# rdevooght/sequence-based-recommendations

Hardware: AMD Instinct MI355X
Metric: user-sequences/sec training (ML-1M shape, seq200 b256) at 1/2/4/8 GPUs (higher is better)
Workload: dtype f32; 1 GPU; c2: train.py -m RNN --r_t GRU --r_l 128 --max_length 200 -b 256 --loss CCE --u_m adam, N=3706 items, Zipf(1.0) ids, lengths=full, 256 rows per GPU; global_batch=256, seq_len=200, parallelism=dp1

## Files before the change

sequence-based-recommendations_amd/csrc/sbr_api.hip:

```cpp
#include "sbr_common.h"
#include <stdarg.h>
#include <stdio.h>
#include <string.h>
#include <algorithm>
#include <stdlib.h>
#include <math.h>
#include <array>
#include <atomic>
#include <chrono>

static thread_local std::string g_err;
void sbr_set_error(const char* fmt, ...) {
    char buf[1024];
    va_list ap; va_start(ap, fmt); vsnprintf(buf, sizeof(buf), fmt, ap); va_end(ap);
    g_err = buf;
}
extern "C" const char* sbr_last_error(void) { return g_err.c_str(); }
extern "C" int sbr_abi_version(void) { return SBR_ABI_VERSION; }


int sbr_build_layout(const sbr_config& cfg, Layout& lay, std::string& err) {
    char buf[256];
#define LFAIL(...) do { snprintf(buf, sizeof(buf), __VA_ARGS__); err = buf; return SBR_EINVAL; } while (0)
    if (cfg.abi_version != SBR_ABI_VERSION) LFAIL("abi_version %d != %d", cfg.abi_version, SBR_ABI_VERSION);
// ... 590 lines not shown
    if (!h->sw.tail_overlap || y.tail_keys < 2 || y.n_sparse || h->sw.bwd_chunks != 1) return 0;
    if (simple_rec(h) || simple_gemm(h) || (y.cfg.flags & (SBR_FLAG_F32_MFMA | SBR_FLAG_ATOMIC_SCATTER))) return 0;
    RecArgs a; memset(&a, 0, sizeof(a));
    a.cell = y.cfg.cell; a.T = y.T; a.Bp = y.Bp; a.H = y.layer[0].H; a.Hp = y.layer[0].Hp; a.G = y.G; a.clip = y.cfg.grad_clip;
    rec_switches(h, a); a.n_in = y.layer[0].n_in_p;
    a.hs = h->A(y.layer[0].a_hs); a.cs = h->A(y.layer[0].a_cs);
    for (int k = 0; k < 4; ++k) a.g[k] = h->A(y.layer[0].a_g[k]);
    if (!sbr_rec_x6p_tail_ok(a)) return 0;
    int nc = std::min(std::min(y.tail_keys, kTailChunksMax), y.T / 16);
    if (nc < 2) return 0;
    const int ch = (y.T + nc - 1) / nc;
    nc = (y.T + ch - 1) / ch;
    if (nc < 2) return 0;
    *ch_out = ch;
    const double geom = sbr_tail_geom(h->sw.tail_scatter_lds);
    SbrTChunks& tc = h->tail_bounds;
    tc.n = nc;
    tc.lo[0] = 0;
    double pw = h->sw.tail_scatter_lds ? (double)kTailFirst : 1.0;
    for (int c = 0; c < nc; ++c) {
        const int rem = y.T - tc.lo[c], left = nc - c;
        const int share = (rem + left - 1) / left;
        const int n_small = nc >= 4 ? nc / 2 : (nc - 1) / 2;
        int sz = (geom > 1.0 && c < n_small) ? std::min(share, std::max(1, (int)(pw + 0.5))) : (geom > 1.0 ? share : std::min(rem, ch));
        if (c == nc - 1) sz = rem;
        sz = std::max(1, std::min(sz, rem - (left - 1)));
        tc.lo[c + 1] = tc.lo[c] + sz;
        pw *= geom > 1.0 ? geom : 1.0;
    }
    for (int c = nc; c <= SBR_TCHUNKS_MAX; ++c) tc.lo[c] = y.T;
    return nc;
}

static int tail_cost_scan(sbr_handle* h) {
    const Layout& y = h->lay;
    h->tail_cost_scanned = false;
    if (!h->sw.tail_scatter_lds) return SBR_OK;
    hipError_t e = hipSuccess;
    if (launch_scatter_cost_scan(h->side2, (const int*)h->A(y.a_soff), (int*)h->A(y.a_sP), y.cfg.input_size, h->tail_nc, y.T * y.Bp * y.F,
                                 y.G * y.layer[0].Hp, kTailScatterUnits, &e)) {
        if (e != hipSuccess) { sbr_set_error("HIP launch failed: %s", hipGetErrorString(e)); return SBR_EHIP; }
        h->tail_cost_scanned = true;
    }
    return SBR_OK;
}

static inline void chain_mark(sbr_handle* h, hipStream_t st, int dir, int which) {
    if (!h->chain_timing || h->ch_n >= sbr_handle::kChain) return;
    hipEvent_t& e = h->ev_ch[h->ch_n][which];
    if (!e && hipEventCreate(&e) != hipSuccess) { e = nullptr; return; }
    (void)hipEventRecord(e, st);
    if (which == 1) { h->ch_dir[h->ch_n] = (unsigned char)dir; h->ch_n += 1; }
}
#define SBR_LAUNCH_CHAIN(DIR, STREAM, CALL) do { chain_mark(h, STREAM, DIR, 0); SBR_LAUNCH(CALL); chain_mark(h, STREAM, DIR, 1); } while (0)

static inline void mark_on(sbr_handle* h, int i, hipStream_t st) {
    if (i == 0) h->marks_shared = 0;
    if ((h->marks_shared >> i) & 1) return;
    if (h->timing && ((h->timing_marks >> i) & 1) && h->ev[h->ring_cur][i]) (void)hipEventRecord(h->ev[h->ring_cur][i], st);
}
static inline void mark(sbr_handle* h, int i) { mark_on(h, i, h->stream); }
static inline hipEvent_t record_shared(sbr_handle* h, hipEvent_t plain, int mk) {
    if (mk >= 0 && h->timing && ((h->timing_marks >> mk) & 1) && h->ev[h->ring_cur][mk]) {
        (void)hipEventRecord(h->ev[h->ring_cur][mk], h->stream);
        h->marks_shared |= 1u << mk;
        return h->ev[h->ring_cur][mk];
// ... 207 lines not shown
    return h->A(ly.a_hs) + (size_t)y.T * y.Bp * ly.Hp;
}

static int side_join(sbr_handle* h) {
    if (h->tail_join_pending) {
        SBR_HIP(hipStreamWaitEvent(h->stream, h->ev_tail2, 0));
        SBR_HIP(hipStreamWaitEvent(h->stream, h->ev_tail, 0));
        h->tail_join_pending = false; h->side_pending = false;
    }
    if (h->side_pending) {
        SBR_HIP(hipEventRecord(h->ev_join, h->side));
        SBR_HIP(hipStreamWaitEvent(h->stream, h->ev_join, 0));
        h->side_pending = false;
    }
    return SBR_OK;
}

extern "C" int sbr_loss_backward_output(sbr_handle* h) {
    CHECK_ARG(h, "null handle");
    sbr_gemm_set_exact_f32((h->lay.cfg.flags & SBR_FLAG_F32_MFMA) != 0);
    if (!h->fwd_done) { sbr_set_error("sbr_loss_backward_output: call sbr_forward first"); return SBR_ESTATE; }
    const Layout& y = h->lay; hipStream_t s = h->stream, sd = h->side;
    const int R = h->n_rows, Hp = y.HLt, N = y.N;
    const bool sg = simple_gemm(h);
    h->grads_clean = false;
    h->dh_slabs_n = 0;
    float* hl = h_last(h);
    float* ws = h->A(y.a_ws);
    float* ws2 = h->A(y.a_ws2);
    const int* tgt = h->btgt;
    if (R < y.Bp) SBR_HIP(hipMemsetAsync(h->A(y.a_dhlast), 0, (size_t)y.Bp * Hp * sizeof(float), s));
    h->side_pending = true;
    h->fill_done = false;
    bool fill_needed = false;
    if (!simple_rec(h))
        for (int l = 0; l < y.L * y.D; ++l) fill_needed = fill_needed || sbr_rec_cluster_ok(rec_args(h, l));
    auto side_batch_work = [&]() -> int {
        if (fill_needed) {
            for (int l = 0; l < y.L * y.D; ++l) {
                RecArgs a = rec_args(h, l);
                if (sbr_rec_cluster_ok(a)) SBR_LAUNCH(sbr_rec_bwd_cl_fill(sd, a));
            }
            SBR_HIP(hipEventRecord(h->ev_fill, sd)); h->fill_done = true;
        }
        if (h->tail_nc >= 2) {
            if (h->ev_lg_rec) SBR_HIP(hipStreamWaitEvent(h->side2, h->ev_lg_rec, 0));
            if (!h->tail_sorted) {
                SBR_LAUNCH(launch_scatter_sort(h->side2, h->bX, h->blen, y.T, y.Bp, y.F, y.cfg.input_size, (int*)h->A(y.a_scnt),
                                               (int*)h->A(y.a_soff), (int*)h->A(y.a_scur), (int*)h->A(y.a_sid), (int*)h->A(y.a_spos), 0,
                                               h->tail_ch, h->tail_nc, &h->tail_bounds, &h->scnt_zero_n));
                { const int rc = tail_cost_scan(h); if (rc != SBR_OK) return rc; }
            }
        } else if (!(y.cfg.flags & SBR_FLAG_ATOMIC_SCATTER) || y.E || y.n_sparse) {
            SBR_LAUNCH(launch_scatter_sort(sd, h->bX, h->blen, y.T, y.Bp, y.F,
                                           y.cfg.input_size, (int*)h->A(y.a_scnt), (int*)h->A(y.a_soff), (int*)h->A(y.a_scur),
                                           (int*)h->A(y.a_sid), (int*)h->A(y.a_spos), y.E ? 1 : 0, 0, 1, nullptr, &h->scnt_zero_n));
            if (y.D == 2 && !y.E)
                SBR_LAUNCH(launch_scatter_sort(sd, (const int*)h->A(y.a_Xr), h->blen, y.T, y.Bp, y.F, y.cfg.input_size,
                                               (int*)h->A(y.a_s2cnt), (int*)h->A(y.a_s2off), (int*)h->A(y.a_s2cur),
                                               (int*)h->A(y.a_s2sid), (int*)h->A(y.a_s2pos), 0));
            SBR_HIP(hipEventRecord(h->ev_sort, sd));
        }
        return SBR_OK;
    };
    if (fill_needed) {
        SBR_HIP(hipEventRecord(h->ev_fork, s));
        SBR_HIP(hipStreamWaitEvent(sd, h->ev_fork, 0));
        const int rc = side_batch_work(); if (rc != SBR_OK) return rc;
    }
    if (y.cfg.loss == SBR_LOSS_CCE || SBR_LOSS_IS_MARGIN(y.cfg.loss)) {
        float* lg = h->A(y.a_logits);
        const int Nl = (N + 3) & ~3;
        const bool bf16p = (y.cfg.flags & SBR_FLAG_BF16_PROJECTION) && !sg;
        int keep = 0;
        bool fold = false;
        if (!sg && y.D == 1 && R == y.Bp && !simple_rec(h)) {
            RecArgs ra = rec_args(h, y.L - 1);
            fold = sbr_rec_x6p_ok(ra) && !sbr_rec_cluster_ok(ra);
        }
        bool head_done = false;
        if (h->sw.head_fuse && y.cfg.loss == SBR_LOSS_CCE && !sg && !bf16p && !(y.cfg.flags & SBR_FLAG_F32_MFMA) && y.D == 1 && R == y.Bp) {
            int nsl = 0; hipError_t he = hipSuccess;
            h->head_epoch += 1; if (!h->head_epoch) h->head_epoch = 1;
            if (launch_head_cce(s, hl, h->P(y.p_WoutT), h->P(y.p_bout), tgt, h->bpop, lg, h->A(y.a_rowcost), ws, y.ws_floats,
                                (unsigned*)h->A(y.a_hstat), (int*)h->A(y.a_fault), y.Bp, N, Nl, Hp, y.Bg, h->head_epoch, h->sw.head_wait_ticks, &nsl, &he,
                                (y.cfg.flags & SBR_FLAG_PROFILE_REC) && (size_t)y.Bp * 16 >= 256 * 8 ? (unsigned long long*)h->A(y.a_prof) + (size_t)2 * (y.Bp / 16) * 16 * 8 : nullptr)) {
                SBR_LAUNCH(he);
                head_done = true;
                if (fold) keep = nsl;
                else SBR_LAUNCH(launch_splitk_reduce(s, ws, nsl, y.Bp, Hp, h->A(y.a_dhlast), Hp, nullptr));
            }
        }
        if (!head_done) {
        if (bf16p) sbr_gemm_set_planes(1);
        else if (layer_gemm_f16(h, false)) sbr_gemm_hint(2, 1.0f, 1.0f);
        const hipError_t ge = launch_gemm(s, hl, Hp, 1, h->P(y.p_WoutT), 1, Hp, lg, Nl, R, N, Hp, nullptr, nullptr, 0, sg);
        sbr_gemm_set_planes(3);
        SBR_LAUNCH(ge);
        if (SBR_LOSS_IS_MARGIN(y.cfg.loss))
            SBR_LAUNCH(launch_margin_loss(s, lg, h->P(y.p_bout), tgt, y.NT, h->bX, h->blen, y.T, y.F, h->A(y.a_dflt), h->A(y.a_rowcost), R, N, Nl,
                                          y.Bg, y.cfg.loss, y.cfg.balance, y.cfg.unique));
        else
        SBR_LAUNCH(launch_softmax_cce(s, lg, h->P(y.p_bout), tgt, h->bpop, h->A(y.a_rowcost), R, N, Nl, y.Bg));
        SBR_LAUNCH(launch_gemm(s, lg, Nl, 1, h->P(y.p_WoutT), Hp, 1, h->A(y.a_dhlast), Hp, R, Hp, N, nullptr, ws, y.ws_floats, sg, 0, 0,
                               fold ? &keep : nullptr));
        }
        h->dh_slabs_n = keep;
        h->ev_lg_rec = record_shared(h, h->ev_lg, 3); h->lg_seq = h->batch_seq;
        SBR_HIP(hipStreamWaitEvent(sd, h->ev_lg_rec, 0));
        if (!fill_needed) { const int rc = side_batch_work(); if (rc != SBR_OK) return rc; }
        h->out_stepped = false;
        const bool will_step_here = h->in_train_step && !y.n_sparse && !sg && h->tail_nc == 0;
        if (h->sw.out_fuse && will_step_here && y.cfg.regularization == 0.0f && y.D == 1) {
            hipError_t oe = hipSuccess;
            float* s1e = y.n_state_arrays > 1 ? h->St(1, 0) : nullptr;
            if (launch_out_grad_step(sd, lg, hl, h->A(y.a_rowcost), h->cost_ptr(), y.cfg.updater, h->P(y.p_WoutT), h->St(0, y.p_WoutT),
                                     s1e ? s1e + y.p_WoutT : nullptr, h->P(y.p_bout), h->St(0, y.p_bout), s1e ? s1e + y.p_bout : nullptr,
                                     R, N, Nl, Hp, y.cfg.learning_rate, y.cfg.rho, y.cfg.beta1, y.cfg.beta2, (long)h->step_count + 1, &oe)) {
                SBR_LAUNCH(oe);
                h->out_stepped = true;
            }
        }
        if (!h->out_stepped) {
        SBR_LAUNCH(launch_sum_cost(sd, h->A(y.a_rowcost), R, h->cost_ptr()));
        const float reg = y.cfg.regularization * (float)R / (float)y.Bg;
        SBR_LAUNCH(launch_colsum_bias(sd, lg, R, N, Nl, h->Gd(y.p_bout), h->P(y.p_bout), reg, h->cost_ptr(), h->A(y.a_csum)));
        SBR_LAUNCH(launch_gemm(sd, lg, 1, Nl, hl, Hp, 1, h->Gd(y.p_WoutT), Hp, N, Hp, R, nullptr, ws2, y.ws2_floats, sg));
        }
        SBR_HIP(hipEventRecord(h->ev_og, sd)); h->og_recorded = true;
        if (h->in_train_step && !y.n_sparse && h->tail_nc == 0 && !simple_gemm(h)) {
            float* s1e = y.n_state_arrays > 1 ? h->St(1, 0) : nullptr;
            if (!h->out_stepped)
            SBR_LAUNCH(launch_update(sd, y.cfg.updater, h->P(y.p_split), h->Gd(y.p_split), h->St(0, y.p_split), s1e ? s1e + y.p_split : nullptr,
                                     y.n_params - y.p_split, y.cfg.learning_rate, y.cfg.rho, y.cfg.beta1, y.cfg.beta2, (long)h->step_count + 1));
            h->out_early = true;
        }
    } else {
        const int C = y.C;
        int* cells = (int*)h->A(y.a_cells);
        float *Wc = h->A(y.a_Wc), *bc = h->A(y.a_bc), *act = h->A(y.a_act), *dWc = h->A(y.a_dWc), *dbc = h->A(y.a_dbc);
        if (h->cells_early) SBR_HIP(hipStreamWaitEvent(s, h->ev_cells, 0));
        else {
        SBR_LAUNCH(launch_build_cells(s, tgt, h->bsmp, y.Bg, y.S, cells));
        if (sparse_lazy(h))
            for (int b = 0; b < y.n_sparse; ++b)
                if (y.sparse[b].kind == 1)
                    SBR_LAUNCH(launch_sparse_catch_up_list(s, sparse_rows(h, b), sparse_upd(h), cells, nullptr, C, C, (int)h->step_count));
        }
        h->cells_early = false;
        SBR_LAUNCH(launch_gather_rows(s, h->P(y.p_WoutT), h->P(y.p_bout), cells, C, Hp, Wc, bc));
        bool head1 = false;
        if (head_sampled_taken(h, R)) {
            hipError_t he = hipSuccess;
            head1 = launch_head_sampled(s, hl, Wc, bc, h->bpop, act, h->A(y.a_rowcost), h->A(y.a_dhlast), R, C, Hp, y.Bg, y.S,
                                        y.cfg.row_offset, y.cfg.loss, y.Bg, &he,
                                        (y.cfg.flags & SBR_FLAG_PROFILE_REC) ? (unsigned long long*)h->A(y.a_prof) + (size_t)2 * (y.Bp / 16) * 16 * 8 : nullptr);
            if (head1) SBR_LAUNCH(he);
        }
        if (!head1) {
        SBR_LAUNCH(launch_gemm(s, hl, Hp, 1, Wc, 1, Hp, act, C, R, C, Hp, nullptr, nullptr, 0, sg));
        SBR_LAUNCH(launch_sampled_loss(s, act, bc, h->bpop, h->A(y.a_rowcost), R, y.Bg, y.S, y.cfg.row_offset,
                                       y.cfg.loss, y.Bg));
        }
        if (!head1) SBR_LAUNCH(launch_gemm(s, act, C, 1, Wc, Hp, 1, h->A(y.a_dhlast), Hp, R, Hp, C, nullptr, nullptr, 0, sg));
        h->ev_lg_rec = record_shared(h, h->ev_lg, 3); h->lg_seq = h->batch_seq;
        SBR_HIP(hipStreamWaitEvent(sd, h->ev_lg_rec, 0));
        SBR_LAUNCH(launch_sum_cost(sd, h->A(y.a_rowcost), R, h->cost_ptr()));
        SBR_LAUNCH(launch_colsum_bias(sd, act, R, C, C, dbc, nullptr, 0.0f, nullptr, h->A(y.a_csum)));
        SBR_LAUNCH(launch_gemm(sd, act, 1, C, hl, Hp, 1, dWc, Hp, C, Hp, R, nullptr, nullptr, 0, sg));
        SBR_LAUNCH(launch_scatter_cells(sd, h->Gd(y.p_WoutT), h->Gd(y.p_bout), dWc, dbc, cells, C, Hp));
        SBR_HIP(hipEventRecord(h->ev_og, sd)); h->og_recorded = true;
        if (!fill_needed) {
            const int rc = side_batch_work(); if (rc != SBR_OK) return rc;
        }
        h->wout_early = false;
        if (h->in_train_step && h->sw.sparse_out_early)
            for (int b = 0; b < y.n_sparse; ++b)
                if (y.sparse[b].kind == 1 && !h->sp_exchanged[b]) {
                    SBR_HIP(hipStreamWaitEvent(sd, h->ev_og, 0));
                    SBR_LAUNCH(launch_sparse_step_list(sd, sparse_rows(h, b), sparse_upd(h), (const int*)h->A(y.a_cells), nullptr, C, C,
                                                       (int)h->step_count + 1));
                    h->wout_early = true;
                }
    }
    mark(h, 3);
    if (h->deferred_join && !h->in_train_step) {
        SBR_HIP(hipEventRecord(h->ev_lg, s));
        SBR_HIP(hipStreamWaitEvent(sd, h->ev_lg, 0));
        return SBR_OK;
    }
    if (!h->in_train_step) return side_join(h);
    return SBR_OK;
}

extern "C" int sbr_backward_recurrent(sbr_handle* h) {
    CHECK_ARG(h, "null handle");
    sbr_gemm_set_exact_f32((h->lay.cfg.flags & SBR_FLAG_F32_MFMA) != 0);
    if (!h->fwd_done) { sbr_set_error("sbr_backward_recurrent: call sbr_forward first"); return SBR_ESTATE; }
    const Layout& y = h->lay; hipStream_t s = h->stream, sd = h->side;
// ... 12 lines not shown
            if (l == y.L - 1) SBR_HIP(hipStreamWaitEvent(s, h->ev_fill, 0));
        }
        a.dh_last = l == y.L - 1 ? h->A(y.a_dhlast) : nullptr;
        if (l == y.L - 1 && h->dh_slabs_n > 0) { a.dh_slabs = ws; a.n_dh_slabs = h->dh_slabs_n; }
        a.dh_ext = l < y.L - 1 ? h->A(ly.a_dhext) : nullptr;
        if (a.prof) a.prof += (size_t)(y.Bp / 16) * 16 * 8;
        const int nblk = sbr_rec_bwd_blocks(a, simple_rec(h));
        const size_t slab = (size_t)ly.Hp * GHp;
        int nc = (sbr_rec_bwd_chunkable(a, simple_rec(h)) && y.T >= 64 && !sg) ? h->sw.bwd_chunks : 1;
        int nsl = (int)std::min<size_t>(kWgradSlices / nc, y.ws2_floats / (slab * nc));
        if (nsl < 1) nc = 1;
        const bool side_wgrad = !simple_rec(h) && !sg && nsl >= 1;
        const bool wg_gemm = (!(y.cfg.flags & SBR_FLAG_F32_MFMA) && ly.Hp >= 96) || !(ly.Hp == 32 || ly.Hp == 64 || ly.Hp == 128);
        const bool wg_f16 = h->sw.wgrad_f16 && !a.relu && y.cfg.grad_clip > 0.0f && y.cfg.grad_clip <= 100.0f;
        if (wg_gemm && nsl > 1) {
            nsl = std::max(1, std::min(nsl, kWgradX6Wgs / (((ly.Hp + 127) / 128) * ((GHp + 127) / 128)) / nc));
        }
        const bool swap = side_wgrad && nc == 1 && y.L == 1 && !y.E && !y.n_sparse &&
                          y.n_params <= ((size_t)4 << 20) &&
                          !(y.cfg.flags & SBR_FLAG_ATOMIC_SCATTER);
        hipStream_t sw = swap ? s : sd;
        hipStream_t sm = swap ? sd : s;
        if (l == 0 && y.L == 1 && h->tail_nc >= 2) {
            const int tnc = h->tail_nc, CH = h->tail_ch;
            const bool serial = h->sw.tail_overlap == 2;
            hipStream_t s2 = serial ? s : h->side2;
            if (serial) {
                sd = s;
                { const int rc = side_join(h); if (rc != SBR_OK) return rc; }
                SBR_HIP(hipEventRecord(h->ev_tail2, h->side2));
                SBR_HIP(hipStreamWaitEvent(s, h->ev_tail2, 0));
            }
            const bool gru = y.cfg.cell == SBR_CELL_GRU;
            int* words = (int*)h->A(y.a_prog);
            const int nwaves = (y.Bp / a.rpt) * 8;
            int* done = (int*)h->A(y.a_done);
            h->prog_epoch = (h->prog_epoch + 1) & 0x7FFFF; if (!h->prog_epoch) h->prog_epoch = 1;
            a.progress = words; a.prog_every = kTailPubEvery; a.prog_epoch = h->prog_epoch;
            const int K = y.T * y.Bp;
            const int cap = (int)std::min<size_t>(256, y.ws2_floats / slab);
            SbrPoll pl{words, nwaves, done, a.prog_epoch, y.Bp, a.fault, 0, 0, h->tail_trace, nullptr, 0};
            if (h->tail_slab_key[0] != K || h->tail_slab_key[1] != cap || !h->tail_slab_dev) {
                sbr_tail_slab_table(K, y.Bp, 255, kTailSlabGrowth, kTailSlabMax, h->tail_slab_host);
                if (!h->tail_slab_dev) SBR_HIP(hipMalloc(&h->tail_slab_dev, 260 * sizeof(int)));
                SBR_HIP(hipMemcpy(h->tail_slab_dev, h->tail_slab_host.data(), h->tail_slab_host.size() * sizeof(int), hipMemcpyHostToDevice));
                h->tail_slab_key[0] = K; h->tail_slab_key[1] = cap;
            }
            pl.slab_lo = h->tail_slab_dev;
            pl.n_slabs = (int)h->tail_slab_host.size() - 1;
            const int n_slabs = std::max(1, std::min(std::min(kTailGemmGroups, cap), pl.n_slabs));
            const bool upd_here = h->in_train_step;
            float* s1a = y.n_state_arrays > 1 ? h->St(1, 0) : nullptr;
            auto upd_on = [&](hipStream_t st, size_t lo, size_t hi, size_t gap_at = (size_t)-1, size_t gap_len = 0) -> hipError_t {
                return launch_update(st, y.cfg.updater, h->P(lo), h->Gd(lo), h->St(0, lo), s1a ? s1a + lo : nullptr, hi - lo - gap_len,
                                     y.cfg.learning_rate, y.cfg.rho, y.cfg.beta1, y.cfg.beta2, (long)h->step_count + 1, gap_at, gap_len);
            };
            if (!serial) a.fence_kb = kTailFenceKb;
            SBR_LAUNCH_CHAIN(1, s, launch_rec_backward(s, a, false));
            mark(h, 4);
            const bool out_early = upd_here && (y.cfg.loss == SBR_LOSS_CCE || SBR_LOSS_IS_MARGIN(y.cfg.loss));
            if (out_early && !h->out_stepped)
                SBR_LAUNCH(upd_on(sd, y.p_split, y.n_params));
            const bool mon_in_units = !serial && h->tail_cost_scanned;
            if (!mon_in_units) SBR_LAUNCH(launch_tail_monitor(serial ? s : h->side3, pl, a.t_lo));
            SBR_LAUNCH(launch_tail_gate(sd, words, nwaves, a.prog_epoch, y.T, a.fault));
            {
                hipError_t we = hipSuccess;
                if (!launch_gemm_slabs_x6_poll(sd, h->A(ly.a_hs), 1, ly.Hp, a.dxt, GHp, 1, ly.Hp, GHp, K, ws2, n_slabs, GHp, slab,
                                               gru ? a.dhi : nullptr, ly.Hp, gru ? 2 * ly.Hp : 0, &we, wg_f16 ? 2 : 3, 1.0f, wg_f16 ? 512.0f : 1.0f, pl)) {
                    sbr_set_error("overlapped tail: the weight-gradient GEMM rejected the shape"); return SBR_EINVAL;
                }
                SBR_LAUNCH(we);
            }
            if (!serial) SBR_LAUNCH(launch_tail_gate(s2, words, nwaves, a.prog_epoch, y.T, a.fault));
            hipError_t se = hipSuccess;
            if (h->tail_cost_scanned && launch_scatter_lds_poll(s2, h->Gd(ly.p_Win), a.dxt, (const int*)h->A(y.a_sid), (const int*)h->A(y.a_spos),
                                                               (const int*)h->A(y.a_soff), (const int*)h->A(y.a_sP), y.cfg.input_size, tnc,
                                                               y.T * y.Bp * y.F, GHp, pl, h->tail_bounds, kTailScatterUnits, &se,
                                                               mon_in_units, a.t_lo)) {
                SBR_LAUNCH(se); h->last_scatter_form = 5;
            } else {
            h->last_scatter_form = 4;
            SBR_LAUNCH(launch_scatter_reduce_poll(s2, h->Gd(ly.p_Win), a.dxt, (const int*)h->A(y.a_sid), (const int*)h->A(y.a_spos),
                                                  (const int*)h->A(y.a_soff), y.cfg.input_size, tnc, CH, y.T * y.Bp * y.F, GHp, y.Bp, pl,
                                                  0, &h->tail_bounds, kTailShortChunks, !serial && kTailFenceKb > 0));
            }
            if (upd_here) SBR_LAUNCH(upd_on(s2, ly.p_Win, ly.p_b));
            SBR_HIP(hipEventRecord(h->ev_tail2, s2));
            if (upd_here && ly.p_peep - ly.p_Whid == slab && (slab & 3) == 0) {
                SBR_LAUNCH(launch_update_from_slabs(sd, y.cfg.updater, ws2, n_slabs, h->P(ly.p_Whid), h->St(0, ly.p_Whid),
                                                    s1a ? s1a + ly.p_Whid : nullptr, slab, y.cfg.learning_rate, y.cfg.rho, y.cfg.beta1,
                                                    y.cfg.beta2, (long)h->step_count + 1));
            } else {
                SBR_LAUNCH(launch_splitk_reduce(sd, ws2, n_slabs, ly.Hp, GHp, h->Gd(ly.p_Whid), GHp, nullptr));
                if (upd_here) SBR_LAUNCH(upd_on(sd, ly.p_Whid, ly.p_peep));
            }
            SBR_HIP(hipEventRecord(h->ev_tail, sd));
            SBR_LAUNCH(launch_rec_reduce_partials(s, a.part, nblk, y.G, ly.Hp, y.cfg.cell, h->Gd(ly.p_b), h->Gd(ly.p_peep),
                                                  h->Gd(ly.p_cinit), h->Gd(ly.p_hinit)));
            mark(h, 5);
            if (upd_here) {
                if (!out_early && h->og_recorded) SBR_HIP(hipStreamWaitEvent(s, h->ev_og, 0));
                SBR_LAUNCH(upd_on(s, ly.p_b, out_early ? y.p_split : y.n_params, ly.p_Whid - ly.p_b, ly.p_peep - ly.p_Whid));
                h->tail_updated = true;
            }
            if (h->deferred_join && !h->in_train_step && !serial) {
                h->tail_join_pending = true;
// ... 628 lines not shown
    SBR_HIP(hipEventSynchronize(e1));
    float ms = 0.f;
    SBR_HIP(hipEventElapsedTime(&ms, e0, e1));
    *us = ms * 1000.0f / (float)reps;
    (void)hipEventDestroy(e0); (void)hipEventDestroy(e1);
    if (entries || rows) {
        std::vector<int> off((size_t)y.cfg.input_size + 1);
        SBR_HIP(hipMemcpy(off.data(), h->A(y.a_soff), off.size() * sizeof(int), hipMemcpyDeviceToHost));
        int64_t nr = 0;
        for (int i = 0; i < y.cfg.input_size; ++i) nr += off[i + 1] > off[i];
        if (entries) *entries = off[y.cfg.input_size];
        if (rows) *rows = nr;
    }
    SBR_HIP(hipMemsetAsync(dW, 0, (size_t)y.cfg.input_size * GHp * sizeof(float), s));
    SBR_HIP(hipStreamSynchronize(s));
    h->tail_sorted = false;
    return SBR_OK;
}

extern "C" int sbr_query(sbr_handle* h, const char* what, int64_t* value) {
    CHECK_ARG(h && what && value, "null argument");
    const Layout& y = h->lay; const std::string w(what);
    if (w == "fused_gather") {
        RecArgs a = rec_args(h, 0);
        *value = (y.E == 0 && y.F == 1 && h->sw.fuse_gather && sbr_rec_fwd_can_fuse_gather(a, simple_rec(h))) ? 1 : 0;
    } else if (w == "rows_per_workgroup") *value = h->rpt;
    else if (w == "head_fused") {
        int cc = 0, cw = 0; size_t lds = 0;
        *value = (h->sw.head_fuse && y.cfg.loss == SBR_LOSS_CCE && !simple_gemm(h) && !(y.cfg.flags & (SBR_FLAG_BF16_PROJECTION | SBR_FLAG_F32_MFMA)) &&
                  y.D == 1 && y.B == y.Bp && sbr_head_plan(y.Bp, y.N, y.HLt, &cc, &cw, &lds) && (size_t)cc * y.Bp * y.HLt <= y.ws_floats) ? cc : 0;
    }
    else if (w == "head_sampled") *value = head_sampled_taken(h, y.B) ? 1 : 0;
    else if (w == "scatter_form") *value = h->last_scatter_form;
    else if (w == "rank_select") *value = h->last_rank_select;
    else if (w == "rank_sort") *value = h->last_rank_sort;
    else if (w == "row_aware_update") *value = h->last_row_aware ? 1 : 0;
    else if (w == "cluster") { RecArgs a = rec_args(h, (y.L - 1) * y.D); *value = (!simple_rec(h) && sbr_rec_cluster_ok(a)) ? 1 : 0; }
    else if (w == "rec_kernel") {
        RecArgs a = rec_args(h, (y.L - 1) * y.D);
        *value = simple_rec(h) ? 0 : sbr_rec_cluster_ok(a) ? 1 : sbr_rec_x6p_ok(a) ? 2 : sbr_rec_x6q_ok(a) ? 3 : 4;
    }
    else if (w.rfind("rec_products_", 0) == 0 || w.rfind("rec_rows_", 0) == 0 || w.rfind("rec_workgroups_", 0) == 0) {
        const bool bwd = w.size() > 4 && w.compare(w.size() - 4, 4, "_bwd") == 0;
        RecArgs a = rec_args(h, (y.L - 1) * y.D);
        const bool cl = !simple_rec(h) && sbr_rec_cluster_ok(a), xp = sbr_rec_x6p_ok(a), xq = sbr_rec_x6q_ok(a);
        const bool x6 = cl || xp || xq || (!a.f32_mfma && (a.Hp == 32 || a.Hp == 64 || a.Hp == 128));
        int products = 0, rows = 16, wgs = y.Bp / 16;
        if (!simple_rec(h) && x6) {
            const bool f16 = (xp || cl || xq) && (bwd ? sbr_rec_f16_bwd(a) : sbr_rec_f16_fwd(a));
            products = f16 ? (xp && !cl ? sbr_rec_x6p_f16_terms() : 3) : 6;
            if (cl && sbr_rec_c16_ok(a)) { rows = 16; wgs = (y.Bp / 16) * (a.Hp / 16); }
            else if (cl) { rows = bwd ? sbr_rec_cluster_bwd_rows(a) : SBR_CL_ROWS; wgs = (y.Bp / rows) * (a.Hp == 256 ? 8 : 32); }
            else { rows = a.rpt; wgs = y.Bp / a.rpt; }
        }
        *value = w.rfind("rec_products_", 0) == 0 ? products : w.rfind("rec_rows_", 0) == 0 ? rows : wgs;
    }
    else if (w == "tail_chunks") { int ch = 0; *value = tail_plan(h, &ch); }
    else if (w == "tail_streams") { int ch = 0; *value = (tail_plan(h, &ch) >= 2 && h->sw.tail_overlap == 1) ? 1 : 0; }
    else if (w == "tail_last_steps") { int ch = 0; *value = tail_plan(h, &ch) >= 2 ? h->tail_bounds.lo[1] : 0; }
    else if (w == "side_stream2") *value = (int64_t)(intptr_t)h->side2;
    else if (w == "tail_chain_cycles" || w == "tail_chain_ticks") {
        unsigned long long c[2] = {0, 0};
        const int nwaves = (y.Bp / h->rpt) * 8;
        SBR_HIP(hipStreamSynchronize(h->stream));
        SBR_HIP(hipMemcpy(c, (const int*)h->A(y.a_prog) + nwaves + 128, sizeof(c), hipMemcpyDeviceToHost));
        *value = (int64_t)c[w == "tail_chain_cycles" ? 0 : 1];
// ... 57 lines not shown
```

sequence-based-recommendations_amd/csrc/sbr_batch.hip:

```cpp
#include "sbr_common.h"
#include <algorithm>
#include <unordered_map>

struct sbr_dataset {
    int64_t n_users, nnz; int n_items;
    hipStream_t stream;
    int* d_items; long long* d_off;
    float* d_popdb; double* d_cdf;
    int* d_rate;
    int shuffle_targets;
    int *d_items_n, *d_rate_n, *d_len_n; int noised; int64_t max_len;
    std::vector<int> len_n32;
    std::vector<int64_t> len_cur;
    int host_rows, hr_targets; uint64_t hr_seed, hr_pass;
    std::vector<float> keep_prob;
    std::vector<int> h_items, h_items_cur;
    std::vector<int64_t> h_off;
    std::vector<int> hr_user, hr_split, hr_tgt, hr_pu, hr_ps, hr_pt;
    int *d_hr_user, *d_hr_split, *d_hr_tgt; size_t cap_hru, cap_hrs, cap_hrt;
    std::vector<int64_t> len;
    std::vector<int> pend_user, pend_k;
    std::vector<int> seg_user, seg_k, seg_row0, seg_batch, batch_begin;
    int *d_seg_user, *d_seg_k, *d_seg_row0, *d_batch_begin; size_t cap_su, cap_sk, cap_sr, cap_bb;
    int *d_split, *d_rowuser; size_t cap_rows;
// ... 527 lines not shown
    if ((r = upload(&d->d_seg_k, &d->cap_sk, d->seg_k, d->stream)) != SBR_OK) return r;
    if ((r = upload(&d->d_seg_row0, &d->cap_sr, d->seg_row0, d->stream)) != SBR_OK) return r;
    if ((r = upload(&d->d_batch_begin, &d->cap_bb, d->batch_begin, d->stream)) != SBR_OK) return r;
    SBR_HIP(hipStreamSynchronize(d->stream));
    d->n_batches = nb; *n_batches = nb;
    return SBR_OK;
}

extern "C" int sbr_dataset_plan_segments(sbr_dataset* d, int64_t* n_segments, const int32_t** seg_user, const int32_t** seg_k,
                                         const int32_t** seg_row0, const int32_t** seg_batch) {
    CHECK_ARG(d && n_segments, "null argument");
    *n_segments = (int64_t)d->seg_user.size();
    if (seg_user) *seg_user = d->seg_user.data();
    if (seg_k) *seg_k = d->seg_k.data();
    if (seg_row0) *seg_row0 = d->seg_row0.data();
    if (seg_batch) *seg_batch = d->seg_batch.data();
    return SBR_OK;
}

extern "C" int sbr_build_batch(sbr_handle* h, sbr_dataset* d, int64_t batch, uint64_t seed) {
    CHECK_ARG(h && d, "null handle / dataset");
    const Layout& y = h->lay;
    CHECK_ARG(y.F == 1 || (y.F == 2 && d->d_rate && y.cfg.input_size == y.N + 10),
              "the native batch builder covers the item index and, with ratings attached (sbr_dataset_set_options), the rating index");
    CHECK_ARG(d->n_items == y.N && (y.cfg.input_size == y.N || y.F == 2), "dataset has %d items, the model %d", d->n_items, y.N);
    CHECK_ARG(!d->shuffle_targets || y.NT <= 16 || d->host_rows, "shuffled targets: at most 16 targets per row on the device");
    CHECK_ARG(d->batch_size == y.Bg, "the pass was planned for batches of %d rows, the model's global batch is %d", d->batch_size, y.Bg);
    CHECK_ARG(batch >= 0 && batch < d->n_batches, "batch %lld outside the planned pass [0,%lld)", (long long)batch, (long long)d->n_batches);
    CHECK_ARG(d->stream == h->stream, "dataset and engine must share one stream");
    hipStream_t s = h->s_bb;
    const int set = h->bb_set ^ 1;
    if (h->train_fwd_open) h->bb_slow = 2;
    if (h->bb_unread && h->bb_slow == 0) h->bb_slow = 1;
    if (h->bb_slow == 0 && h->ev_lg_rec && h->lg_seq > h->set_use[set]) {
        SBR_HIP(hipStreamWaitEvent(s, h->ev_lg_rec, 0));
    } else {
        hipStream_t all[4] = {h->stream, h->side, h->side2, h->side3};
        for (hipStream_t q : all) { SBR_HIP(hipEventRecord(h->ev_bbw, q)); SBR_HIP(hipStreamWaitEvent(s, h->ev_bbw, 0)); }
        if (h->bb_slow > 0) --h->bb_slow;
    }
    if ((size_t)y.Bg > d->cap_rows) {
        (void)hipFree(d->d_split); (void)hipFree(d->d_rowuser); d->d_split = d->d_rowuser = nullptr;
        SBR_HIP(hipMalloc(&d->d_split, (size_t)y.Bg * sizeof(int)));
        SBR_HIP(hipMalloc(&d->d_rowuser, (size_t)y.Bg * sizeof(int)));
        d->cap_rows = y.Bg;
    }
    const unsigned long long sd = seed ^ (0x9E3779B97F4A7C15ull * (unsigned long long)(batch + 1));
    const int* len_n = d->noised ? d->d_len_n : nullptr;
    const int* src_items = d->noised ? d->d_items_n : d->d_items;
    const int* src_rate = d->noised && d->d_rate ? d->d_rate_n : d->d_rate;
    const int *split = d->d_split, *rowuser = d->d_rowuser, *tgtpos = nullptr;
    if (d->host_rows) {
        CHECK_ARG(d->hr_targets == y.NT, "the rows were planned for %d targets, the model has %d", d->hr_targets, y.NT);
        split = d->d_hr_split + batch * y.Bg; rowuser = d->d_hr_user + batch * y.Bg; tgtpos = d->d_hr_tgt + batch * (int64_t)y.Bg * y.NT;
    } else {
        const int sb = d->batch_begin[batch], se = d->batch_begin[batch + 1];
        bb_split_kernel<<<se - sb, 256, 0, s>>>(d->d_off, len_n, d->d_seg_user, d->d_seg_k, d->d_seg_row0, sb, sd, d->d_split, d->d_rowuser);
        SBR_LAUNCH(hipGetLastError());
    }
    int *bX = (int*)h->A(set ? y.a_X2 : y.a_X), *blen = (int*)h->A(set ? y.a_len2 : y.a_len), *btgt = (int*)h->A(set ? y.a_tgt2 : y.a_tgt);
    int* bsmp = (int*)h->A(set ? y.a_smp2 : y.a_smp);
    float* bpop = h->A(set ? y.a_pop2 : y.a_pop);
    const bool sampled = y.S > 0;
    const int tgt_rows = sampled ? y.Bg : y.B, tgt_offset = sampled ? 0 : y.cfg.row_offset;
    const int extra = (tgt_rows * y.NT + 63) / 64 + (y.S + 63) / 64;
    bb_pack_kernel<<<y.Bp + extra, 64, 0, s>>>(src_items, src_rate, d->d_off, len_n, split, rowuser, d->d_popdb, d->d_cdf, d->n_items, y.T,
                                                y.F, y.NT, d->shuffle_targets, y.cfg.row_offset, y.B, y.Bp, tgt_rows, tgt_offset, y.S, sd, bX,
                                                blen, btgt, bpop, bsmp, tgtpos);
// ... 9 lines not shown
```

sequence-based-recommendations_amd/csrc/sbr_common.h:

```cpp
#pragma once
#include <hip/hip_runtime.h>
#include <stdint.h>
#include <stddef.h>
#include <string>
#include <vector>
#include "../../include/sbr_rnn.h"

#define SBR_BWD_CHUNKS 4
#define SBR_ALIGN_FLOATS 64

static inline size_t sbr_align(size_t n_floats) { return (n_floats + SBR_ALIGN_FLOATS - 1) / SBR_ALIGN_FLOATS * SBR_ALIGN_FLOATS; }
static inline int sbr_gates(int cell) { return cell == SBR_CELL_LSTM ? 4 : (cell == SBR_CELL_GRU ? 3 : 1); }
static inline int sbr_pad_hidden(int H) {
    if (H <= 16) return 16;
    if (H <= 32) return 32;
    if (H <= 64) return 64;
    if (H <= 128) return 128;
    if (H <= 256) return 256;
    if (H <= 512) return 512;
    return (H + 63) / 64 * 64;
}

struct LayerLayout {
    int H, Hp, G;
// ... 73 lines not shown
    size_t a_X2, a_len2, a_tgt2, a_smp2, a_pop2;
    size_t a_scnt, a_soff, a_scur, a_sid, a_spos;
    size_t a_sP;
    size_t a_hstat;
    size_t a_srpart, a_srid; int sr_slots;
    int tail_keys;
    size_t a_prog;
    size_t a_done;
};

int sbr_build_layout(const sbr_config& cfg, Layout& lay, std::string& err);

struct ParamDesc { std::string name; int layer; int kind; int gate; int64_t d0, d1; int ndim; };
void sbr_param_descs(const Layout& lay, std::vector<ParamDesc>& out);

#define SBR_TCHUNKS_MAX 9
struct SbrTChunks { int n; int lo[SBR_TCHUNKS_MAX + 1]; };
static inline SbrTChunks sbr_uniform_tchunks(int tch, int n) {
    SbrTChunks tc; tc.n = tch > 0 ? n : 0;
    for (int c = 0; c <= SBR_TCHUNKS_MAX; ++c) tc.lo[c] = tch * (c < n ? c : n);
    return tc;
}
constexpr int kWgradSlices = 256;
constexpr int kWgradX6Wgs = 512;
constexpr int kTailChunksMax = 8;
constexpr int kTailPubEvery = 2;
constexpr int kTailShortChunks = 3;
constexpr int kTailFenceKb = 124;
constexpr int kTailFirst = 6;
constexpr int kTailScatterUnits = 192;
constexpr int kTailGemmGroups = 64;
constexpr int kTailSlabMax = 512;
constexpr double kTailSlabGrowth = 0.35;
static inline double sbr_tail_geom(int scatter_lds) { return scatter_lds ? 1.6 : 2.6; }
constexpr int kRankThreads = 1024;
constexpr int kRankLdsRow = 32768;
constexpr int kRankSortLds = 2048;

#define HEAD_WAIT_TICKS 6000ull
struct SbrSwitches {
    int rpt = 0;
    int bwd_chunks = 1;
    int cluster = 1;
    int cl_linear = 0;
    int cl16 = 1;
    int c16_two_level = 1;
    int x6_pipe = 1;
    int x6_f16 = 1;
    int x6_f16_bwd = 1;
    int fuse_gather = 1;
    int gemm_f16 = 1;
    int wgrad_f16 = 1;
    int tail_overlap = 1;
    int tail_scatter_lds = 1;
    int tail_trace = 0;
    int scat_range = 1;
    int sparse_out_early = 1;
    int head_fuse = 1;
    unsigned long long head_wait_ticks = HEAD_WAIT_TICKS;
    int out_fuse = 1;
    int row_aware = 1;
};

struct sbr_handle {
    Layout lay;
    SbrSwitches sw;
// ... 18 lines not shown
    int dh_slabs_n = 0;
    std::vector<ParamDesc> descs;
    int rpt = 16;
    int cl_epoch = 0;
    int sp_exchanged[2] = {0, 0};
    int sp_ncand[2] = {0, 0};
    int sp_epoch = 0;
    float* lag_host = nullptr;
    unsigned lag_seq[2] = {0, 0}, lag_counter = 0;
    int lag_slot = 0, lag_pending = -1;
    const int *bX = nullptr, *blen = nullptr, *btgt = nullptr, *bsmp = nullptr; const float* bpop = nullptr;
#ifndef SBR_BB_STREAM
#define SBR_BB_STREAM 0
#endif
    hipStream_t s_bb = nullptr;
    int bb_set = 0;
    uint64_t batch_seq = 0;
    uint64_t set_use[2] = {0, 0};
    uint64_t lg_seq = 0;
    bool bb_unread = false;
    bool train_fwd_open = false;
    int bb_slow = 0;
    int n_rows = 0;
    int64_t step_count = 0;
    bool have_batch = false, fwd_done = false;
    bool grads_clean = false;
    bool timing = false;
    unsigned timing_marks = 0;
    int tail_nc = 0, tail_ch = 0;
    SbrTChunks tail_bounds = {};
    unsigned long long* tail_trace = nullptr;
    bool tail_sorted = false;
    void* rank_scratch = nullptr; size_t rank_scratch_bytes = 0; int last_rank_select = 0, last_rank_sort = 0;
    int last_scatter_form = -1; bool last_row_aware = false;
    bool tail_cost_scanned = false;
    int scnt_zero_n = 0;
    std::vector<int> tail_slab_host; int* tail_slab_dev = nullptr; int tail_slab_key[2] = {0, 0};
    int prog_epoch = 0;
    bool tail_updated = false;
    bool tail_join_pending = false;
    bool step_open = false;
    hipEvent_t ev_lg_rec = nullptr;
    bool tail_swapped = false;
    unsigned marks_shared = 0;
    static const int kRing = 64;
    hipEvent_t ev[kRing][SBR_N_PHASES] = {};
    int ring_used = 0;
    int ring_cur = 0;
    static const int kChain = 256;
    hipEvent_t ev_ch[kChain][2] = {};
    unsigned char ch_dir[kChain] = {};
    int ch_n = 0;
    bool chain_timing = false;
    float* P(size_t off) const { return arena + lay.s_params + off; }
    float* Gd(size_t off) const { return arena + lay.s_grads + off; }
    float* St(int k, size_t off) const { return arena + lay.s_state + (size_t)k * lay.n_params + off; }
    float* A(size_t off) const { return arena + lay.s_act + off; }
    float* cost_ptr() const { return arena + lay.s_grads + lay.n_params; }
};

void sbr_set_error(const char* fmt, ...);
#define SBR_HIP(call) do { hipError_t e_ = (call); if (e_ != hipSuccess) { \
    sbr_set_error("%s failed: %s (%s:%d)", #call, hipGetErrorString(e_), __FILE__, __LINE__); return SBR_EHIP; } } while (0)

#define CHECK_ARG(cond, ...) do { if (!(cond)) { sbr_set_error(__VA_ARGS__); return SBR_EINVAL; } } while (0)
#define SBR_LAUNCH(call) do { hipError_t e_ = (call); if (e_ != hipSuccess) { \
    sbr_set_error("%s failed: %s (%s:%d)", #call, hipGetErrorString(e_), __FILE__, __LINE__); return SBR_EHIP; } } while (0)

#define SBR_DYN_LDS(KERNEL, LDS) do { static int sbr_dyn_lds_set_ = -1; if ((int)(LDS) > sbr_dyn_lds_set_) { \
        (void)hipFuncSetAttribute((const void*)KERNEL, hipFuncAttributeMaxDynamicSharedMemorySize, (int)(LDS)); sbr_dyn_lds_set_ = (int)(LDS); } } while (0)
#define SBR_DONE_COPIES 32
#define SBR_DONE_STRIDE 1088
struct SbrPoll { const int* words; int n; int* done; int epoch; int rows_per_step; int* fault; int n_small, k_small;
                 unsigned long long* trace; const int* slab_lo; int n_slabs; };

hipError_t launch_gather_xt(hipStream_t s, const float* Win, const float* bias, const int* X, float* xt,
                            int T, int Bp, int F, int GHp, int n_rows_in);
hipError_t launch_scatter_rows(hipStream_t s, float* dWin, const float* dxt, const int* X, const int* len,
                               int T, int Bp, int F, int GHp);
hipError_t launch_scatter_sort(hipStream_t s, const int* X, const int* len, int T, int Bp, int F, int n_ids, int* cnt,
                               int* offs, int* cur, int* sid, int* spos, int concat = 0, int tch = 0, int n_tchunks = 1, const SbrTChunks* bounds = nullptr,
                               int* cnt_zero_n = nullptr);
int sbr_scatter_lds_ids();
hipError_t launch_tail_gate(hipStream_t s, const int* progress, int n, int epoch, int target, int* fault);
hipError_t launch_gather_concat(hipStream_t s, const float* Wemb, const int* X, float* out, int T, int Bp, int F, int Ep);
hipError_t launch_rev_rows_int(hipStream_t s, const int* X, const int* len, int* Xr, int T, int Bp, int F);
hipError_t launch_rev_rows(hipStream_t s, const float* src, const int* len, float* dst, int T, int Bp, int W);
hipError_t launch_cat_outputs(hipStream_t s, const float* hs_f, const float* hs_b, const int* len, float* cat, int T, int Bp, int Hp);
hipError_t launch_hcat(hipStream_t s, const float* hf, const float* hb, float* out, int Bp, int Hp);
hipError_t launch_split_cols(hipStream_t s, const float* src, float* a, float* b, int rows, int Hp);
hipError_t launch_uncat(hipStream_t s, const float* f, const float* r, const int* len, float* out_f, float* out_b, int T, int Bp,
                        int W, int Hp);
bool launch_scatter_range(hipStream_t s, float* dWin, const float* dxt, const int* sid, const int* spos, const int* offs, int n_ids,
                          int GHp, float* part, int* part_id, int n_ranges, hipError_t* err);
#define SBR_SCAT_RANGES 512
bool launch_scatter_wide(hipStream_t s, float* dWin, const float* dxt, const int* sid, const int* spos, const int* offs, int n_ids,
                         int max_entries, int GHp, float* part, int* aux, int n_slots, hipError_t* err);
struct SbrScatStep { float* p; float* s0; float* s1; int* last; int updater, t_to; float lr, rho, b1, b2, a_t; };
static inline int sbr_scatter_wide_slots(size_t max_entries) { return (int)(max_entries / 64 + max_entries / 65 + 2); }
hipError_t launch_scatter_reduce(hipStream_t s, float* dWin, const float* dxt, const int* sid, const int* spos,
                                 const int* offs, int n_ids, int max_entries, int GHp, int Bp, int key_lo = 0, bool accumulate = false, int acc_chunk = 32);
bool launch_scatter_cost_scan(hipStream_t s, const int* offs, int* P, int n_ids, int n_tchunks, int max_entries, int GHp, int units,
                              hipError_t* err);
hipError_t launch_tail_monitor(hipStream_t s, const SbrPoll& poll, int t_lo);
bool launch_scatter_lds_poll(hipStream_t s, float* dWin, const float* dxt, const int* sid, const int* spos, const int* offs, const int* P,
                             int n_ids, int n_tchunks, int max_entries, int GHp, const SbrPoll& poll, const SbrTChunks& bounds,
                             int units, hipError_t* err, bool monitor = false, int t_lo = 0);
hipError_t launch_scatter_reduce_poll(hipStream_t s, float* dWin, const float* dxt, const int* sid, const int* spos, const int* offs,
                                      int n_ids, int n_tchunks, int tch, int max_entries, int GHp, int Bp, const SbrPoll& poll, int first_key = 0, const SbrTChunks* bounds = nullptr, int short_chunks = 0, bool fence_on = false);

__host__ __device__ __forceinline__ size_t sbr_blocked_index(int t, int row, int col, int Bp, int ncols) {
    return (((size_t)t * (Bp >> 4) + (row >> 4)) * (ncols >> 4) + (col >> 4)) * 256 + (row & 15) * 16 + (col & 15);
}

struct RecArgs {
    int cell, T, Bp, H, Hp, G;
    float clip;
// ... 153 lines not shown
```

sequence-based-recommendations_amd/csrc/sbr_misc.hip:

```cpp
#include "sbr_common.h"
#include "sbr_rec_p.h"
#include <math.h>

typedef float f32x4 __attribute__((ext_vector_type(4)));

__device__ __forceinline__ float wave_sum(float v) {
#pragma unroll
    for (int o = 32; o > 0; o >>= 1) v += __shfl_xor(v, o);
    return v;
}
__device__ __forceinline__ float wave_max(float v) {
#pragma unroll
    for (int o = 32; o > 0; o >>= 1) v = fmaxf(v, __shfl_xor(v, o));
    return v;
}
__device__ __forceinline__ float block_sum(float v, float* red) {
    v = wave_sum(v);
    __syncthreads();
    if ((threadIdx.x & 63) == 0) red[threadIdx.x >> 6] = v;
    __syncthreads();
    float s = 0.0f;
    for (int w = 0; w < (int)(blockDim.x >> 6); ++w) s += red[w];
    return s;
}
// ... 1127 lines not shown
    }
#define SR(NV) do { if ((accumulate || key_lo) && chunk == 16) scat_reduce_kernel<NV, 16, true><<<grid, 256, 0, s>>>((const f32x4*)dxt, sid, spos, offs, n_ids, dWin, R4, Bp, key_lo); \
                    else if (accumulate || key_lo) scat_reduce_kernel<NV, 32, true><<<grid, 256, 0, s>>>((const f32x4*)dxt, sid, spos, offs, n_ids, dWin, R4, Bp, key_lo); \
                    else if (chunk == 16) scat_reduce_kernel<NV, 16><<<grid, 256, 0, s>>>((const f32x4*)dxt, sid, spos, offs, n_ids, dWin, R4, Bp); \
                    else if (chunk == 32) scat_reduce_kernel<NV, 32><<<grid, 256, 0, s>>>((const f32x4*)dxt, sid, spos, offs, n_ids, dWin, R4, Bp); \
                    else scat_reduce_kernel<NV, 64><<<grid, 256, 0, s>>>((const f32x4*)dxt, sid, spos, offs, n_ids, dWin, R4, Bp); } while (0)
    if (accumulate || key_lo) { if (nv <= 1) SR(1); else if (nv <= 2) SR(2); else if (nv <= 4) SR(4); else return hipErrorInvalidValue; }
    else if (nv <= 1) SR(1); else if (nv <= 2) SR(2); else if (nv <= 4) SR(4); else if (nv <= 8) SR(8); else if (nv <= 16) SR(16);
    else return hipErrorInvalidValue;
#undef SR
    return hipGetLastError();
}

__global__ void __launch_bounds__(512) tail_gate_kernel(const int* __restrict__ progress, int n, int epoch, int target, int* __restrict__ fault) {
    for (int i = threadIdx.x; i < n; i += blockDim.x) {
        const unsigned long long t0 = wall_clock64();
        for (;;) {
            const int v = __hip_atomic_load(progress + i, __ATOMIC_RELAXED, __HIP_MEMORY_SCOPE_AGENT);
            if ((v >> 12) == epoch && (v & 0xfff) <= target) break;
            if (wall_clock64() - t0 > SBR_POLL_TICKS) { atomicOr(fault, 8); break; }
            __builtin_amdgcn_s_sleep(8);
        }
    }
}

__global__ void __launch_bounds__(256) tail_monitor_kernel(SbrPoll pl, int t_lo) { tail_monitor_loop(pl, t_lo); }
hipError_t launch_tail_monitor(hipStream_t s, const SbrPoll& poll, int t_lo) {
    tail_monitor_kernel<<<1, 256, 0, s>>>(poll, t_lo);
    return hipGetLastError();
}

hipError_t launch_tail_gate(hipStream_t s, const int* progress, int n, int epoch, int target, int* fault) {
    tail_gate_kernel<<<1, 512, 0, s>>>(progress, n, epoch, target, fault);
    return hipGetLastError();
}

__global__ void scatter_rows_kernel(float* __restrict__ dWin, const f32x4* __restrict__ dxt, const int* __restrict__ X,
                                    const int* __restrict__ len, int T, int Bp, int F, int R4) {
    const size_t total = (size_t)T * Bp * R4;
    for (size_t i = (size_t)blockIdx.x * blockDim.x + threadIdx.x; i < total; i += (size_t)gridDim.x * blockDim.x) {
        const int f4 = (int)(i % R4);
        const size_t pos = i / R4;
        const int b = (int)(pos % Bp), t = (int)(pos / Bp);
        if (t >= len[b]) continue;
        const f32x4 v = dxt[i];
        const int* ids = X + ((size_t)b * T + t) * F;
        for (int f = 0; f < F; ++f) {
            float* dst = dWin + ((size_t)ids[f] * R4 + f4) * 4;
            atomicAdd(dst + 0, v[0]); atomicAdd(dst + 1, v[1]); atomicAdd(dst + 2, v[2]); atomicAdd(dst + 3, v[3]);
        }
    }
}

hipError_t launch_scatter_rows(hipStream_t s, float* dWin, const float* dxt, const int* X, const int* len, int T,
                               int Bp, int F, int GHp) {
    const int R4 = GHp / 4;
    const size_t total = (size_t)T * Bp * R4;
    const int grid = (int)min((size_t)256 * 16, (total + 255) / 256);
    scatter_rows_kernel<<<grid, 256, 0, s>>>(dWin, (const f32x4*)dxt, X, len, T, Bp, F, R4);
    return hipGetLastError();
}

__global__ void __launch_bounds__(256) softmax_cce_kernel(float* __restrict__ logits, const float* __restrict__ bout,
                                                          const int* __restrict__ target, const float* __restrict__ pop,
                                                          float* __restrict__ rowcost, int N, long ld, int Bglobal) {
    __shared__ float red[4];
// ... 578 lines not shown
```

Measured before the change: 794,500 user-sequences/s.

## Gate side stream on tail progress words instead of logits event

Instead of recording an event after the output-layer gradient and making the side stream wait on it, the side stream now launches a single-wave polling gate that spins on device progress words published by the recurrent backward tail. The tail reuses the same epoch, so side work can be queued early and released by device-side progress rather than a stream dependency. The second gate on the scatter stream also becomes a lighter one-wave kernel. This removes a cross-stream event wait and aims to overlap side work sooner, at the cost of a persistent spinning wave, a timeout/fault risk if progress words are never published, and more complex epoch bookkeeping.

```diff
diff --git a/sequence-based-recommendations_amd/csrc/sbr_api.hip b/sequence-based-recommendations_amd/csrc/sbr_api.hip
--- a/sequence-based-recommendations_amd/csrc/sbr_api.hip
+++ b/sequence-based-recommendations_amd/csrc/sbr_api.hip
@@ -646,6 +646,15 @@
     return nc;
 }
 
+static int tail_next_epoch(sbr_handle* h) {
+    h->prog_epoch = (h->prog_epoch + 1) & 0x7FFFF; if (!h->prog_epoch) h->prog_epoch = 1;
+    return h->prog_epoch;
+}
+static int* tail_words(sbr_handle* h, int* nwaves) {
+    *nwaves = (h->lay.Bp / rec_args(h, 0).rpt) * 8;
+    return (int*)h->A(h->lay.a_prog);
+}
+
 static int tail_cost_scan(sbr_handle* h) {
     const Layout& y = h->lay;
     h->tail_cost_scanned = false;
@@ -919,6 +928,7 @@
     if (R < y.Bp) SBR_HIP(hipMemsetAsync(h->A(y.a_dhlast), 0, (size_t)y.Bp * Hp * sizeof(float), s));
     h->side_pending = true;
     h->fill_done = false;
+    h->tail_gated = false; h->last_tail_gated = 0;
     bool fill_needed = false;
     if (!simple_rec(h))
         for (int l = 0; l < y.L * y.D; ++l) fill_needed = fill_needed || sbr_rec_cluster_ok(rec_args(h, l));
@@ -955,6 +965,20 @@
         SBR_HIP(hipStreamWaitEvent(sd, h->ev_fork, 0));
         const int rc = side_batch_work(); if (rc != SBR_OK) return rc;
     }
+    auto release_side = [&]() -> int {
+        const bool mark3 = h->timing && ((h->timing_marks >> 3) & 1) && h->ev[h->ring_cur][3];
+        if (kTailGateFirst && h->in_train_step && h->tail_nc >= 2 && h->sw.tail_overlap == 1 && h->tail_sorted && y.L == 1 && y.D == 1 && !fill_needed && !mark3) {
+            int nwaves = 0;
+            int* words = tail_words(h, &nwaves);
+            SBR_LAUNCH(launch_tail_gate_wave(sd, words, nwaves, tail_next_epoch(h), y.T, (int*)h->A(y.a_fault)));
+            h->tail_gated = true;
+            h->ev_lg_rec = nullptr; h->ev_step_rec = h->ev_fork; h->lg_seq = h->batch_seq;
+        } else {
+            h->ev_lg_rec = h->ev_step_rec = record_shared(h, h->ev_lg, 3); h->lg_seq = h->batch_seq;
+            SBR_HIP(hipStreamWaitEvent(sd, h->ev_lg_rec, 0));
+        }
+        return SBR_OK;
+    };
     if (y.cfg.loss == SBR_LOSS_CCE || SBR_LOSS_IS_MARGIN(y.cfg.loss)) {
         float* lg = h->A(y.a_logits);
         const int Nl = (N + 3) & ~3;
@@ -993,8 +1017,7 @@
                                fold ? &keep : nullptr));
         }
         h->dh_slabs_n = keep;
-        h->ev_lg_rec = record_shared(h, h->ev_lg, 3); h->lg_seq = h->batch_seq;
-        SBR_HIP(hipStreamWaitEvent(sd, h->ev_lg_rec, 0));
+        { const int rc = release_side(); if (rc != SBR_OK) return rc; }
         if (!fill_needed) { const int rc = side_batch_work(); if (rc != SBR_OK) return rc; }
         h->out_stepped = false;
         const bool will_step_here = h->in_train_step && !y.n_sparse && !sg && h->tail_nc == 0;
@@ -1050,8 +1073,7 @@
                                        y.cfg.loss, y.Bg));
         }
         if (!head1) SBR_LAUNCH(launch_gemm(s, act, C, 1, Wc, Hp, 1, h->A(y.a_dhlast), Hp, R, Hp, C, nullptr, nullptr, 0, sg));
-        h->ev_lg_rec = record_shared(h, h->ev_lg, 3); h->lg_seq = h->batch_seq;
-        SBR_HIP(hipStreamWaitEvent(sd, h->ev_lg_rec, 0));
+        { const int rc = release_side(); if (rc != SBR_OK) return rc; }
         SBR_LAUNCH(launch_sum_cost(sd, h->A(y.a_rowcost), R, h->cost_ptr()));
         SBR_LAUNCH(launch_colsum_bias(sd, act, R, C, C, dbc, nullptr, 0.0f, nullptr, h->A(y.a_csum)));
         SBR_LAUNCH(launch_gemm(sd, act, 1, C, hl, Hp, 1, dWc, Hp, C, Hp, R, nullptr, nullptr, 0, sg));
@@ -1130,11 +1152,12 @@
                 SBR_HIP(hipStreamWaitEvent(s, h->ev_tail2, 0));
             }
             const bool gru = y.cfg.cell == SBR_CELL_GRU;
-            int* words = (int*)h->A(y.a_prog);
-            const int nwaves = (y.Bp / a.rpt) * 8;
+            int nwaves = 0;
+            int* words = tail_words(h, &nwaves);
             int* done = (int*)h->A(y.a_done);
-            h->prog_epoch = (h->prog_epoch + 1) & 0x7FFFF; if (!h->prog_epoch) h->prog_epoch = 1;
-            a.progress = words; a.prog_every = kTailPubEvery; a.prog_epoch = h->prog_epoch;
+            const bool gated = h->tail_gated && !serial;
+            h->tail_gated = false; h->last_tail_gated = gated;
+            a.progress = words; a.prog_every = kTailPubEvery; a.prog_epoch = gated ? h->prog_epoch : tail_next_epoch(h);
             const int K = y.T * y.Bp;
             const int cap = (int)std::min<size_t>(256, y.ws2_floats / slab);
             SbrPoll pl{words, nwaves, done, a.prog_epoch, y.Bp, a.fault, 0, 0, h->tail_trace, nullptr, 0};
@@ -1161,7 +1184,7 @@
                 SBR_LAUNCH(upd_on(sd, y.p_split, y.n_params));
             const bool mon_in_units = !serial && h->tail_cost_scanned;
             if (!mon_in_units) SBR_LAUNCH(launch_tail_monitor(serial ? s : h->side3, pl, a.t_lo));
-            SBR_LAUNCH(launch_tail_gate(sd, words, nwaves, a.prog_epoch, y.T, a.fault));
+            if (!gated) SBR_LAUNCH(launch_tail_gate(sd, words, nwaves, a.prog_epoch, y.T, a.fault));
             {
                 hipError_t we = hipSuccess;
                 if (!launch_gemm_slabs_x6_poll(sd, h->A(ly.a_hs), 1, ly.Hp, a.dxt, GHp, 1, ly.Hp, GHp, K, ws2, n_slabs, GHp, slab,
@@ -1170,7 +1193,8 @@
                 }
                 SBR_LAUNCH(we);
             }
-            if (!serial) SBR_LAUNCH(launch_tail_gate(s2, words, nwaves, a.prog_epoch, y.T, a.fault));
+            if (gated) SBR_LAUNCH(launch_tail_gate_wave(s2, words, nwaves, a.prog_epoch, y.T, a.fault));
+            else if (!serial) SBR_LAUNCH(launch_tail_gate(s2, words, nwaves, a.prog_epoch, y.T, a.fault));
             hipError_t se = hipSuccess;
             if (h->tail_cost_scanned && launch_scatter_lds_poll(s2, h->Gd(ly.p_Win), a.dxt, (const int*)h->A(y.a_sid), (const int*)h->A(y.a_spos),
                                                                (const int*)h->A(y.a_soff), (const int*)h->A(y.a_sP), y.cfg.input_size, tnc,
@@ -1865,6 +1889,7 @@
     }
     else if (w == "head_sampled") *value = head_sampled_taken(h, y.B) ? 1 : 0;
     else if (w == "scatter_form") *value = h->last_scatter_form;
+    else if (w == "tail_gate_first") *value = h->last_tail_gated;
     else if (w == "rank_select") *value = h->last_rank_select;
     else if (w == "rank_sort") *value = h->last_rank_sort;
     else if (w == "row_aware_update") *value = h->last_row_aware ? 1 : 0;
diff --git a/sequence-based-recommendations_amd/csrc/sbr_batch.hip b/sequence-based-recommendations_amd/csrc/sbr_batch.hip
--- a/sequence-based-recommendations_amd/csrc/sbr_batch.hip
+++ b/sequence-based-recommendations_amd/csrc/sbr_batch.hip
@@ -583,8 +583,8 @@
     const int set = h->bb_set ^ 1;
     if (h->train_fwd_open) h->bb_slow = 2;
     if (h->bb_unread && h->bb_slow == 0) h->bb_slow = 1;
-    if (h->bb_slow == 0 && h->ev_lg_rec && h->lg_seq > h->set_use[set]) {
-        SBR_HIP(hipStreamWaitEvent(s, h->ev_lg_rec, 0));
+    if (h->bb_slow == 0 && h->ev_step_rec && h->lg_seq > h->set_use[set]) {
+        SBR_HIP(hipStreamWaitEvent(s, h->ev_step_rec, 0));
     } else {
         hipStream_t all[4] = {h->stream, h->side, h->side2, h->side3};
         for (hipStream_t q : all) { SBR_HIP(hipEventRecord(h->ev_bbw, q)); SBR_HIP(hipStreamWaitEvent(s, h->ev_bbw, 0)); }
diff --git a/sequence-based-recommendations_amd/csrc/sbr_common.h b/sequence-based-recommendations_amd/csrc/sbr_common.h
--- a/sequence-based-recommendations_amd/csrc/sbr_common.h
+++ b/sequence-based-recommendations_amd/csrc/sbr_common.h
@@ -129,6 +129,8 @@
 constexpr int kTailGemmGroups = 64;
 constexpr int kTailSlabMax = 512;
 constexpr double kTailSlabGrowth = 0.35;
+constexpr bool kTailGateFirst = true;
+constexpr int kTailGateSleep = 32;
 static inline double sbr_tail_geom(int scatter_lds) { return scatter_lds ? 1.6 : 2.6; }
 constexpr int kRankThreads = 1024;
 constexpr int kRankLdsRow = 32768;
@@ -213,11 +215,14 @@
     unsigned long long* tail_trace = nullptr;
     bool tail_sorted = false;
     void* rank_scratch = nullptr; size_t rank_scratch_bytes = 0; int last_rank_select = 0, last_rank_sort = 0;
+    int last_tail_gated = -1;
     int last_scatter_form = -1; bool last_row_aware = false;
     bool tail_cost_scanned = false;
     int scnt_zero_n = 0;
     std::vector<int> tail_slab_host; int* tail_slab_dev = nullptr; int tail_slab_key[2] = {0, 0};
     int prog_epoch = 0;
+    bool tail_gated = false;
+    hipEvent_t ev_step_rec = nullptr;
     bool tail_updated = false;
     bool tail_join_pending = false;
     bool step_open = false;
@@ -264,6 +269,7 @@
                                int* cnt_zero_n = nullptr);
 int sbr_scatter_lds_ids();
 hipError_t launch_tail_gate(hipStream_t s, const int* progress, int n, int epoch, int target, int* fault);
+hipError_t launch_tail_gate_wave(hipStream_t s, const int* progress, int n, int epoch, int target, int* fault);
 hipError_t launch_gather_concat(hipStream_t s, const float* Wemb, const int* X, float* out, int T, int Bp, int F, int Ep);
 hipError_t launch_rev_rows_int(hipStream_t s, const int* X, const int* len, int* Xr, int T, int Bp, int F);
 hipError_t launch_rev_rows(hipStream_t s, const float* src, const int* len, float* dst, int T, int Bp, int W);
diff --git a/sequence-based-recommendations_amd/csrc/sbr_misc.hip b/sequence-based-recommendations_amd/csrc/sbr_misc.hip
--- a/sequence-based-recommendations_amd/csrc/sbr_misc.hip
+++ b/sequence-based-recommendations_amd/csrc/sbr_misc.hip
@@ -1183,6 +1183,30 @@
 
 hipError_t launch_tail_gate(hipStream_t s, const int* progress, int n, int epoch, int target, int* fault) {
     tail_gate_kernel<<<1, 512, 0, s>>>(progress, n, epoch, target, fault);
+    return hipGetLastError();
+}
+
+__global__ void __launch_bounds__(64) tail_gate_wave_kernel(const int* __restrict__ progress, int n, int epoch, int target, int* __restrict__ fault) {
+    const unsigned long long t0 = wall_clock64();
+    auto passed = [&](int v) { return (v >> 12) == epoch && (v & 0xfff) <= target; };
+    for (;;) {
+        if (passed(__hip_atomic_load(progress, __ATOMIC_RELAXED, __HIP_MEMORY_SCOPE_AGENT))) break;
+        if (wall_clock64() - t0 > SBR_POLL_TICKS) { if (threadIdx.x == 0) atomicOr(fault, 8); return; }
+        __builtin_amdgcn_s_sleep(kTailGateSleep);
+    }
+    for (;;) {
+        bool ok = true;
+#pragma unroll 8
+        for (int i = 0; i < n; i += 64)
+            ok = passed(__hip_atomic_load(progress + min(i + (int)threadIdx.x, n - 1), __ATOMIC_RELAXED, __HIP_MEMORY_SCOPE_AGENT)) && ok;
+        if (__all(ok)) break;
+        if (wall_clock64() - t0 > SBR_POLL_TICKS) { if (threadIdx.x == 0) atomicOr(fault, 8); return; }
+        __builtin_amdgcn_s_sleep(8);
+    }
+}
+hipError_t launch_tail_gate_wave(hipStream_t s, const int* progress, int n, int epoch, int target, int* fault) {
+    if (n < 1) return hipErrorInvalidValue;
+    tail_gate_wave_kernel<<<1, 64, 0, s>>>(progress, n, epoch, target, fault);
     return hipGetLastError();
 }
 
```

After: 821,300 user-sequences/s (median of 6 runs). 3.4% higher.
